# wjwei-handsome/wgatools

Measured on AMD Instinct MI355X. Metric: paf_cigar_ops_per_s (paf2maf+stat), higher is better.
Workload: dtype u8

## Files before the change

wgatools_amd/csrc/wga_intrin.h:

```cpp
#ifndef WGA_INTRIN_H
#define WGA_INTRIN_H

#ifdef WGA_EMU
#include "wga_intrin_emu.h"
#else

#define WGA_UNI32(x) ((u32)__builtin_amdgcn_readfirstlane((int)(x)))
#define WGA_UNI64(x)                                                               \
  (((u64)(u32)__builtin_amdgcn_readfirstlane((int)((u64)(x) >> 32)) << 32) |       \
   (u64)(u32)__builtin_amdgcn_readfirstlane((int)(u32)(u64)(x)))

#ifdef WGA_WAVE_ID_PLAIN
#define WGA_WAVE_ID(t) ((u32)(t) >> 6)
#else
#define WGA_WAVE_ID(t) ((u32)__builtin_amdgcn_readfirstlane((int)((u32)(t) >> 6)))
#endif

#define WGA_PIN(x) asm volatile("" : "+v"(x))
#define WGA_PIN4(a, b, c, d) asm volatile("" : "+v"(a), "+v"(b), "+v"(c), "+v"(d))
#define WGA_PIN7(a, b, c, d, e, f, g) asm volatile("" : "+v"(a), "+v"(b), "+v"(c), "+v"(d), "+v"(e), "+v"(f), "+v"(g))

__device__ __forceinline__ u32 wave_incl_scan_u32(u32 v) {
  v += (u32)__builtin_amdgcn_update_dpp(0, (int)v, 0x111, 0xF, 0xF, false);
  v += (u32)__builtin_amdgcn_update_dpp(0, (int)v, 0x112, 0xF, 0xF, false);
  v += (u32)__builtin_amdgcn_update_dpp(0, (int)v, 0x114, 0xF, 0xF, false);
  v += (u32)__builtin_amdgcn_update_dpp(0, (int)v, 0x118, 0xF, 0xF, false);
  v += (u32)__builtin_amdgcn_update_dpp(0, (int)v, 0x142, 0xA, 0xF, false);
  v += (u32)__builtin_amdgcn_update_dpp(0, (int)v, 0x143, 0xC, 0xF, false);
  return v;
}
__device__ __forceinline__ u32 wave_incl_scan_max_u32(u32 v) {
  u32 t;
  t = (u32)__builtin_amdgcn_update_dpp(0, (int)v, 0x111, 0xF, 0xF, false); v = v > t ? v : t;
  t = (u32)__builtin_amdgcn_update_dpp(0, (int)v, 0x112, 0xF, 0xF, false); v = v > t ? v : t;
  t = (u32)__builtin_amdgcn_update_dpp(0, (int)v, 0x114, 0xF, 0xF, false); v = v > t ? v : t;
  t = (u32)__builtin_amdgcn_update_dpp(0, (int)v, 0x118, 0xF, 0xF, false); v = v > t ? v : t;
  t = (u32)__builtin_amdgcn_update_dpp(0, (int)v, 0x142, 0xA, 0xF, false); v = v > t ? v : t;
  t = (u32)__builtin_amdgcn_update_dpp(0, (int)v, 0x143, 0xC, 0xF, false); v = v > t ? v : t;
  return v;
}
__device__ __forceinline__ u32 wave_shr1_u32(u32 v, u32 fill) {
  return (u32)__builtin_amdgcn_update_dpp((int)fill, (int)v, 0x138, 0xF, 0xF, false);
}
__device__ __forceinline__ u32 wave_last_u32(u32 incl) { return (u32)__builtin_amdgcn_readlane((int)incl, 63); }
template <u32 K>
__device__ __forceinline__ u64 lane_put_u64(u64 v, u64 uniform_val, u32 lane) {
  (void)lane;
  u32 lo = (u32)v, hi = (u32)(v >> 32);
  const u32 ulo = WGA_UNI32((u32)uniform_val), uhi = WGA_UNI32((u32)(uniform_val >> 32));
  asm("v_writelane_b32 %0, %1, %2" : "+v"(lo) : "s"(ulo), "n"(K));
  asm("v_writelane_b32 %0, %1, %2" : "+v"(hi) : "s"(uhi), "n"(K));
  return ((u64)hi << 32) | (u64)lo;
}

__device__ __forceinline__ u32 byte_perm(u32 hi, u32 lo, u32 sel) { return __builtin_amdgcn_perm(hi, lo, sel); }

#define WGA_BUF_OOB 0xFFFFFFFFu
typedef __amdgpu_buffer_rsrc_t BufRsrc;
typedef u32 u32x4_v __attribute__((vector_size(16)));
__device__ __forceinline__ BufRsrc buf_make(const void* base, u32 bytes) {
  const u64 b = (u64)base;
  const u32 lo = (u32)__builtin_amdgcn_readfirstlane((int)(u32)b);
  const u32 hi = (u32)__builtin_amdgcn_readfirstlane((int)(u32)(b >> 32));
  const u32 n = (u32)__builtin_amdgcn_readfirstlane((int)bytes);
  return __builtin_amdgcn_make_buffer_rsrc((void*)(((u64)hi << 32) | (u64)lo), (short)0, (int)n, 0x00020000);
}
__device__ __forceinline__ void buf_load16(const BufRsrc& r, u32 off, u32 v[4]) {
  const u32x4_v x = __builtin_amdgcn_raw_buffer_load_b128(r, (int)off, 0, 0);
  v[0] = x[0];
  v[1] = x[1];
  v[2] = x[2];
  v[3] = x[3];
}
#ifndef WGA_STORE_AUX
#define WGA_STORE_AUX 0
#endif
__device__ __forceinline__ void buf_store16(const BufRsrc& r, u32 off, const u32 v[4]) {
  const u32x4_v x = {v[0], v[1], v[2], v[3]};
  __builtin_amdgcn_raw_buffer_store_b128(x, r, (int)off, 0, WGA_STORE_AUX);
}
#ifndef WGA_STREAM_AUX
#define WGA_STREAM_AUX 2
#endif
__device__ __forceinline__ void buf_store16_stream(const BufRsrc& r, u32 off, const u32 v[4]) {
  const u32x4_v x = {v[0], v[1], v[2], v[3]};
  __builtin_amdgcn_raw_buffer_store_b128(x, r, (int)off, 0, WGA_STREAM_AUX);
}

__device__ __forceinline__ u64 wave_get_u64(u32 v, int k) {
  return (u64)(u32)__builtin_amdgcn_readlane((int)v, k) | ((u64)(u32)__builtin_amdgcn_readlane((int)v, k + 1) << 32);
}
__device__ __forceinline__ u32 wave_get_u32(u32 v, int k) { return (u32)__builtin_amdgcn_readlane((int)v, k); }
__device__ __forceinline__ u32 wave_get_u32_dyn(u32 v, u32 k) { return (u32)__builtin_amdgcn_readlane((int)v, (int)k); }
#define WGA_CLOCK() ((u64)__builtin_amdgcn_s_memtime())
#define WGA_SLEEP(n) __builtin_amdgcn_s_sleep(n)
#define WGA_WAVE_SYNC() __builtin_amdgcn_wave_barrier()

#ifndef WGA_MBCNT
#define WGA_MBCNT 1
#endif
__device__ __forceinline__ u32 lane_rank(u64 m, u32 lane) {
#if WGA_MBCNT
  (void)lane;
  return (u32)__builtin_amdgcn_mbcnt_hi((u32)(m >> 32), __builtin_amdgcn_mbcnt_lo((u32)m, 0u));
#else
  return (u32)__popcll(m & ((1ull << lane) - 1ull));
#endif
}

__device__ __forceinline__ u32x4_a16 ops_load16(const u32* p) {
#ifdef WGA_OPS_NT
  return __builtin_nontemporal_load((const u32x4_a16*)p);
#else
  return *(const u32x4_a16*)p;
#endif
}

__device__ __forceinline__ u32 bit_mask(u32 bits, u32 idx) { return (u32)__builtin_amdgcn_sbfe((int)bits, idx, 1u); }
__device__ __forceinline__ u32 bit_test(u32 bits, u32 idx) { return __builtin_amdgcn_ubfe(bits, idx, 1u); }

#define WGA_KARG_SPACE __attribute__((address_space(4)))
#define WGA_KARG_SEGMENT(T, a) ((T)__builtin_amdgcn_kernarg_segment_ptr())
#define WGA_KARG_FRESH(p) asm volatile("" : "+s"(p))

#ifndef WGA_W_STORE_AUX
#define WGA_W_STORE_AUX 2
#endif
__device__ __forceinline__ void buf_store16_w(const BufRsrc& r, u32 off, const u32 v[4]) {
  const u32x4_v x = {v[0], v[1], v[2], v[3]};
  __builtin_amdgcn_raw_buffer_store_b128(x, r, (int)off, 0, WGA_W_STORE_AUX);
}

__device__ __forceinline__ void lds_dma16(const void* gbase, u32 voff, void* lds_dst) {
  const u64 gb = WGA_UNI64((u64)gbase);
  const u32 ld = WGA_UNI32((u32)(u64)lds_dst);
  u32 keep;
  asm volatile("s_mov_b32 %0, m0\n\ts_mov_b32 m0, %3\n\ts_nop 0\n\tglobal_load_lds_dwordx4 %1, %2\n\ts_mov_b32 m0, %0"
               : "=&s"(keep)
               : "v"(voff), "s"(gb), "s"(ld)
               : "memory");
}
__device__ __forceinline__ void lds_dma16_after_reads(const void* gbase, u32 voff, void* lds_dst) {
  asm volatile("s_waitcnt lgkmcnt(0)" ::: "memory");
  lds_dma16(gbase, voff, lds_dst);
}
__device__ __forceinline__ void gstore16_nt(void* base, u32 voff, const u32 v[4]) {
  const u64 b = WGA_UNI64((u64)base);
  const u32x4_v x = {v[0], v[1], v[2], v[3]};
  asm volatile("global_store_dwordx4 %0, %1, %2 nt" ::"v"(voff), "v"(x), "s"(b) : "memory");
}
__device__ __forceinline__ void vm_wait(u32 k) {
  switch (k) {
    case 0: asm volatile("s_waitcnt vmcnt(0)" ::: "memory"); break;
    case 1: asm volatile("s_waitcnt vmcnt(1)" ::: "memory"); break;
    case 2: asm volatile("s_waitcnt vmcnt(2)" ::: "memory"); break;
    case 3: asm volatile("s_waitcnt vmcnt(3)" ::: "memory"); break;
    case 4: asm volatile("s_waitcnt vmcnt(4)" ::: "memory"); break;
    case 5: asm volatile("s_waitcnt vmcnt(5)" ::: "memory"); break;
    case 6: asm volatile("s_waitcnt vmcnt(6)" ::: "memory"); break;
    case 7: asm volatile("s_waitcnt vmcnt(7)" ::: "memory"); break;
    case 8: asm volatile("s_waitcnt vmcnt(8)" ::: "memory"); break;
    case 9: asm volatile("s_waitcnt vmcnt(9)" ::: "memory"); break;
    case 10: asm volatile("s_waitcnt vmcnt(10)" ::: "memory"); break;
    case 11: asm volatile("s_waitcnt vmcnt(11)" ::: "memory"); break;
    case 12: asm volatile("s_waitcnt vmcnt(12)" ::: "memory"); break;
    case 13: asm volatile("s_waitcnt vmcnt(13)" ::: "memory"); break;
    case 14: asm volatile("s_waitcnt vmcnt(14)" ::: "memory"); break;
    case 15: asm volatile("s_waitcnt vmcnt(15)" ::: "memory"); break;
    default: asm volatile("" ::: "memory"); break;
  }
}
__device__ __forceinline__ u32 bfi_b32(u32 mask, u32 a, u32 b) { return (a & mask) | (b & ~mask); }

#endif

struct wga_u64x2 {
  u64 x, y;
};
#if defined(__HIP_DEVICE_COMPILE__) && !defined(WGA_EMU)
#define WGA_RO_SPACE __attribute__((address_space(4)))
#define WGA_RO32(p) (*(const WGA_RO_SPACE u32*)(u64)(const u32*)(p))
#define WGA_RO64(p) (*(const WGA_RO_SPACE u64*)(u64)(const u64*)(p))
__device__ __forceinline__ wga_u64x2 wga_ro16(const u64* p) {
  typedef u64 u64x2_v __attribute__((vector_size(16)));
  const u64x2_v v = *(const WGA_RO_SPACE u64x2_v*)(u64)p;
  return {v[0], v[1]};
}
#define WGA_RO_HERE2(a, b) asm volatile("" ::"s"(a), "s"(b))
#define WGA_RO_HERE4(a, b, c, d) asm volatile("" ::"s"(a), "s"(b), "s"(c), "s"(d))
#else
#define WGA_RO32(p) (*(const u32*)(p))
#define WGA_RO64(p) (*(const u64*)(p))
__device__ __forceinline__ wga_u64x2 wga_ro16(const u64* p) { return {p[0], p[1]}; }
#define WGA_RO_HERE2(a, b) ((void)0)
#define WGA_RO_HERE4(a, b, c, d) ((void)0)
#endif

#endif
```

wgatools_amd/csrc/wga_kernels_k2s.h:

```cpp
#ifndef WGA_KERNELS_K2S_H
#define WGA_KERNELS_K2S_H

#include "wga_kernels.h"

#define WGA_S_FIFO 320u
#define WGA_S_MAX_JOB_TILES 32u
#define WGA_S_U 4u
#define WGA_S_WAVE_BYTES ((WGA_S_FIFO + 4u) * 8u + 1024u + 1024u + 256u + 272u + 16u)
#ifndef WGA_AUTO_LONG_VARIANT
#define WGA_AUTO_LONG_VARIANT 3
#endif

__global__ __launch_bounds__(256) void k_pseudo_rec_desc(u32 n, const wga_class_sums* sums, const u8* strand_neg, const u64* q_src_off,
                                                         const u64* q_src_len, const u64* skip, const u64* dst_off, const u64* op_off,
                                                         u64 q_fa_bytes, wga_rec_desc* out, u8* tile_flag) {
  const u32 r = blockIdx.x * 256u + threadIdx.x;
  if (r >= n) return;
  const wga_class_sums cs = sums[r];
  wga_rec_desc d;
  d.t_row_off = 0;
  d.q_row_off = dst_off[r] - skip[r];
  d.t_src_off = 0;
  d.t_src_len = skip[r];
  d.q_src_off = q_src_off ? q_src_off[r] : 0ull;
  d.q_src_len = q_src_len ? q_src_len[r] : 0ull;
  d.I_total = cs.i + cs.s;
  d.D_total = cs.d;
  d.L = cs.mx + cs.d;
  const bool clean = !q_src_len || d.q_src_len == cs.mx + cs.i + cs.s;
  const bool inside = !q_src_off || (d.q_src_off >= 32ull && d.q_src_off + d.q_src_len + 32ull <= q_fa_bytes);
  d.neg = (strand_neg[r] != 0 ? 1u : 0u) | (clean ? 0u : 8u);
  out[r] = d;
  if (clean && inside) return;
  const u64 a = op_off[r], b = op_off[r + 1];
  if (b <= a) return;
  for (u64 t = a / WGA_TILE; t <= (b - 1) / WGA_TILE; t++) tile_flag[t] = 1;
}

__device__ __forceinline__ u32 comp4s(u32 x, u32* bad) {
  const u32 sel = x & 0x07070707u;
  const u32 fold = byte_perm(0x474EFF54u, 0x43FF41FFu, sel);
  const u32 comp = byte_perm(0x434E0D41u, 0x47FF54FFu, sel);
  *bad = (x & 0xDFDFDFDFu) ^ fold;
  return comp | (x & 0x20202020u);
}

#define WGA_S_NOINLINE __forceinline__
__device__ WGA_S_NOINLINE void stream_store_bytes(u8* p, u32 o0, u32 o1, u32 o2, u32 o3, int lo, int hi) {
#pragma clang loop vectorize(disable) unroll(disable)
  for (int j = lo; j < hi; j++) {
    const u32 wj = j < 4 ? o0 : j < 8 ? o1 : j < 12 ? o2 : o3;
    p[j] = (u8)(wj >> (8 * (j & 3)));
  }
}
__device__ WGA_S_NOINLINE void stream_report_bad(u64* bad_base_pos, u32 b0, u32 b1, u32 b2, u32 b3, int lo, int hi, u32 Cl,
                                                 i64 Kseg, const u32* fifo, u32 k, u32 nf, u32 adj) {
#pragma clang loop vectorize(disable) unroll(disable)
  for (int j = lo; j < hi; j++) {
    const u32 bw = j < 4 ? b0 : j < 8 ? b1 : j < 12 ? b2 : b3;
    if (((bw >> (8 * (j & 3))) & 0xFFu) == 0u) continue;
    const u32 cj = Cl + (u32)j;
    u32 ad = adj;
    if (fifo) {
      u32 i = k - 1u;
      while (i + 1u < nf && (int)(fifo[2u * (i + 1u)] - cj) <= 0) i++;
      ad = fifo[2u * (i + 1u) + 1u];
    }
    atomicMin(bad_base_pos, (u64)((i64)(u64)(cj - ad) + Kseg));
  }
}

#define WGA_S_PSEUDO 2
#define WGA_S_SYMBOL 3
template <int MODE>
__device__ __forceinline__ u32 stream_glen(u32 c0, u32 c1) {
  return MODE == WGA_S_SYMBOL ? (c1 >> 1) - (c0 >> 1) : MODE == WGA_S_PSEUDO ? ((int)(c1 - c0) > 0 ? c1 - c0 : 0u) : c1 - c0;
}
__device__ __forceinline__ u32 stream_symbol(u32 cu) { return (cu & 1u) ? 0x2D2D2D2Du : 0x30303030u; }
template <int MODE>
__device__ __forceinline__ void stream_row(const ExpandArgs& a, u8* const lds, const u32 lane, const u64 job, const u64 t0,
                                           const u64 t1) {
  const u32 skipm = WGA_RO32(a.job_skip + job);
  u32* const s_fifo = (u32*)lds;
  u32x4_a16* const s_P = (u32x4_a16*)(s_fifo + 2u * (WGA_S_FIFO + 4u));
  u32* const s_q = (u32*)(s_P + 64);
  u32* const s_T = s_q + 256;
  u32x4_a16* const s_lm = (u32x4_a16*)(s_T + 64);
  u64* const s_k = (u64*)(s_lm + 17);
  if (lane < 17u) {
    u32x4_a16 m;
    for (int d = 0; d < 4; d++) m[d] = bytemask(0, (int)lane - 4 * d);
    s_lm[lane] = m;
  }
  constexpr bool QROW = MODE != 0;
  constexpr bool TCOORD = MODE >= WGA_S_PSEUDO;
  constexpr bool SYM = MODE == WGA_S_SYMBOL;
  constexpr u32 COL_MASK = TCOORD ? 0x585u : 0x787u;
  constexpr u32 GAP_MASK = MODE == 0 ? 0x202u : SYM ? 0x504u : 0x404u;
  constexpr u32 SKIP_MASK = MODE == WGA_S_PSEUDO ? 0x212u : 0u;
  const u8* const fa = QROW ? a.q_fa : a.t_fa;
  const u64 fa_bytes = QROW ? a.q_fa_bytes : a.t_fa_bytes;
  const u64 job_lo = t0 * WGA_TILE;
  const u32 q_end = WGA_UNI32((u32)((t1 * WGA_TILE < a.n_ops ? t1 * WGA_TILE : a.n_ops) - job_lo));
  const BufRsrc obuf = buf_make(a.ops + job_lo, (u32)(((a.n_ops - job_lo) < 0x3FFFFFFFull ? (a.n_ops - job_lo) : 0x3FFFFFFFull) * 4ull));

  u32 C_known = 0, cum_known = 0;
  u32 nf = 1;
  u32 e0 = 1;
  u32 pos = 0;
  u32 q = 0;
  u32 q_lo = 0, q_hi = 0;
  u32 rec = 0, re = 0;
  u8* dst_seg = nullptr;
  BufRsrc sbuf = buf_make(fa, 0u);
  u32 S32 = 0;
  bool rc = false;
  bool live = false;
  bool bnd = false;
  bool fin = false;
  u32 C_b = 0, cum_b = 0;
  u32 C_min = 0;
  u64 t = t0;
  u32 ow[4] = {0, 0, 0, 0}, xl0 = 0, xg0 = 0;
  u32 own[4] = {0, 0, 0, 0};

  auto fifo_dedupe = [&]() {
    WGA_WAVE_SYNC();
    u32 n_new = nf;
    if (lane == 0u) {
      u32 w = e0;
      for (u32 r = e0; r < nf; r++) {
        const u32 gs = s_fifo[2u * r], cu = s_fifo[2u * r + 1u];
        const bool dup = w > e0 && s_fifo[2u * (w - 1u)] == gs && (int)(cu - s_fifo[2u * (w - 1u) + 1u]) <= 0 &&
                         (int)(s_fifo[2u * (r + 1u) + 1u] - cu) <= 0;
        if (!dup) {
          s_fifo[2u * w] = gs;
          s_fifo[2u * w + 1u] = cu;
          w++;
        }
      }
      for (u32 k = 0; k < 3u; k++) {
        s_fifo[2u * (w + k)] = s_fifo[2u * (nf + k)];
        s_fifo[2u * (w + k) + 1u] = s_fifo[2u * (nf + k) + 1u];
      }
      n_new = w;
    }
    nf = wave_get_u32(n_new, 0);
    WGA_WAVE_SYNC();
  };

  for (;;) {
    {
      const u32 lim = bnd ? C_b : C_known;
      const bool all = bnd || fin;
      while ((int)(lim - pos) > 0) {
        if (TCOORD && (int)(C_min - pos) > 0) {
          const u32 to = (int)(lim - C_min) > 0 ? C_min : lim;
          u32 c;
          do {
            const u32 idx = e0 + lane < nf ? e0 + lane : nf;
            c = (u32)__popcll(__ballot(idx < nf && (int)(s_fifo[2u * idx] - to) < 0));
            e0 += c;
          } while (c == 64u);
          pos = to;
          continue;
        }
        u8* const A = dst_seg + pos;
        const u32 mis = (u32)(u64)A & 1023u;
        u8* const B = A - mis;
        const u32 room = WGA_S_U * 1024u - mis;
        if (!all && (lim - pos) < room) break;
        const u32 Cs = pos;
        u32 Ce = (lim - pos) < room ? lim : pos + room;
        const u32 Cl0 = Cs - mis;
        if (e0 + 255u < nf) {
          const u32 g255 = WGA_UNI32(s_fifo[2u * (e0 + 255u)]);
          if ((int)(g255 - Ce) < 0) Ce = Cl0 + ((g255 - Cl0) & ~15u);
          if (MODE == WGA_S_PSEUDO && (int)(Ce - Cs) < 16) {
            fifo_dedupe();
            continue;
          }
        }

        s_T[lane] = 0u;
        WGA_WAVE_SYNC();
        u32 nE = 0;
        {
          u32 base = e0, c;
          do {
            const u32 idx = base + lane < nf ? base + lane : nf;
            const u32 gsr = s_fifo[2u * idx] - Cl0;
            const bool in = gsr < Ce - Cl0;
            c = (u32)__popcll(__ballot(in));
            if (in) atomicAdd(&s_T[(gsr >> 4) & 63u], 1u << (8u * (gsr >> 10)));
            base += c;
            nE += c;
          } while (c == 64u);
        }
        WGA_WAVE_SYNC();
        const u32 tw = s_T[lane];
        WGA_WAVE_SYNC();
        const u32 tinc = wave_incl_scan_u32(tw);
        const u32 texc = tinc - tw;
        const u32 ttot = wave_last_u32(tinc);

        u32 kbase = e0;
        u32 qn = 0, rpk = 0, cls = 0;
        u32 adjv[WGA_S_U];
        const u32 wsp = Ce - Cs - 16u, asp = Ce - Cs + 15u;
        const bool any16 = (Ce - Cs) >= 16u;
        u32 qcum = 0;
#pragma unroll
        for (u32 u = 0; u < WGA_S_U; u++) {
          const u32 cnt = (tw >> (8u * u)) & 255u;
          const u32 k = kbase + ((texc >> (8u * u)) & 255u);
          kbase += (ttot >> (8u * u)) & 255u;
          const u32 Cl = Cl0 + 1024u * u + 16u * lane;
          const bool whole = any16 && (Cl - Cs) <= wsp, active = (Cl + 15u - Cs) < asp;
          const u32x4_a1 fe = *(const u32x4_a1*)(s_fifo + 2u * (k - 1u));
          const int rel0 = (int)(fe[0] + stream_glen<MODE>(fe[1], fe[3]) - Cl);
          const bool quiet = whole && cnt == 0u;
          const bool plain = quiet && rel0 <= 0;
          const bool dashes = quiet && rel0 >= 16;
          const bool flagged = active && !(plain || dashes);
          adjv[u] = fe[3];
          cls |= ((plain ? 1u : 0u) | (dashes ? 2u : 0u) | (flagged ? 4u : 0u) | (SYM ? (fe[1] & 1u) << 3 : 0u)) << (4u * u);
          const u64 m = __ballot(flagged);
          if (flagged) {
            const u32 r = qn + lane_rank(m, lane);
            s_q[r & 255u] = (k << 8) | (u << 6) | lane;
            rpk |= (r & 255u) << (8u * u);
          }
          qcum |= (qn > 255u ? 255u : qn) << (8u * u);
          qn += (u32)__popcll(m);
        }
        if (qn > 64u) {
          u32 keep = 1u;
#pragma unroll
          for (u32 u = 2; u <= WGA_S_U; u++) {
            const u32 upto = u == WGA_S_U ? qn : (qcum >> (8u * u)) & 255u;
            const bool sat = u < WGA_S_U && ((qcum >> (8u * u)) & 255u) == 255u;
            if (upto <= 64u && !sat) keep = u;
          }
          const u32 Cn = Cl0 + 1024u * keep;
          if ((int)(Cn - Ce) < 0) Ce = Cn;
          qn = keep == WGA_S_U ? qn : (qcum >> (8u * keep)) & 255u;
          nE = 0;
#pragma unroll
          for (u32 u = 0; u < WGA_S_U; u++)
            if (u < keep) nE += (ttot >> (8u * u)) & 255u;
        }
        const BufRsrc dbuf = buf_make(B, WGA_S_U * 1024u);

        WGA_WAVE_SYNC();
        if (lane < qn) {
          const u32 ent = s_q[lane];
          const u32 k = ent >> 8, Cl = Cl0 + 16u * (ent & 255u);
          int lo = (int)(Cs - Cl), hi = (int)(Ce - Cl);
          lo = lo < 0 ? 0 : (lo > 16 ? 16 : lo);
          hi = hi > 16 ? 16 : (hi < 0 ? 0 : hi);
          const u32x4_a1 ea = *(const u32x4_a1*)(s_fifo + 2u * (k - 1u));
          const u32x4_a1 eb = *(const u32x4_a1*)(s_fifo + 2u * (k + 1u));
          const u32 gs0 = ea[0], cu0 = ea[1], gs1 = ea[2], cu1 = ea[3], gs2 = eb[0], cu2 = eb[1];
          int a1 = (int)(gs0 + stream_glen<MODE>(cu0, cu1) - Cl);
          a1 = a1 < lo ? lo : (a1 > hi ? hi : a1);
          int b1 = (int)(gs1 - Cl);
          b1 = b1 < a1 ? a1 : (b1 > hi ? hi : b1);
          const u32 gl1 = stream_glen<MODE>(cu1, cu2);
          int e1 = gl1 >= 16u ? 16 : b1 + (int)gl1;
          e1 = e1 > hi ? hi : e1;
          bool more = (int)(gs2 - Cl) < hi;
          u32 W0[4], W1[4];
          if (!SYM) {
            buf_load16(sbuf, b1 > a1 ? (rc ? S32 - Cl + cu1 : S32 + Cl - cu1) : WGA_BUF_OOB, W0);
            buf_load16(sbuf, hi > e1 ? (rc ? S32 - Cl + cu2 : S32 + Cl - cu2) : WGA_BUF_OOB, W1);
          }
          const u32x4_a16 La = s_lm[a1], Lb = s_lm[b1], Le = s_lm[e1];
          u32 o[4], bad[4] = {0u, 0u, 0u, 0u};
#pragma unroll
          for (int d = 0; d < 4; d++) {
            if (SYM) {
              o[d] = bfi_b32(La[d], stream_symbol(cu0), bfi_b32(Le[d] & ~Lb[d], stream_symbol(cu1), 0x31313131u));
              continue;
            }
            u32 cp;
            if (rc)
              cp = comp4s(bfi_b32(Lb[d], bswap32(W0[3 - d]), bswap32(W1[3 - d])), &bad[d]);
            else
              cp = bfi_b32(Lb[d], W0[d], W1[d]);
            const u32 md = La[d] | (Le[d] & ~Lb[d]);
            o[d] = bfi_b32(md, 0x2D2D2D2Du, cp);
            bad[d] &= ~md;
          }
          u32 ie = k + 1u;
          while (more) {
            const u32 gsi = s_fifo[2u * ie], cui = s_fifo[2u * ie + 1u], gsn = s_fifo[2u * ie + 2u], cun = s_fifo[2u * ie + 3u];
            const int b = (int)(gsi - Cl);
            const u32 len = stream_glen<MODE>(cui, cun);
            const int e = len >= (u32)(hi - b) ? hi : b + (int)len;
            u32 W[4];
            if (SYM)
              W[0] = W[1] = W[2] = W[3] = 0x31313131u;
            else
              buf_load16(sbuf, rc ? S32 - Cl + cun : S32 + Cl - cun, W);
            const u32x4_a16 Mb = s_lm[b], Me = s_lm[e];
#pragma unroll
            for (int d = 0; d < 4; d++) {
              u32 x = W[d], bw = 0u;
              if (rc) x = comp4s(bswap32(W[3 - d]), &bw);
              if (SYM)
                o[d] = bfi_b32(Mb[d], o[d], bfi_b32(Me[d], stream_symbol(cui), x));
              else
                o[d] = bfi_b32(Mb[d], o[d], bfi_b32(Me[d], 0x2D2D2D2Du, x));
              bad[d] = (bad[d] & Mb[d]) | (bw & ~Me[d]);
            }
            ie++;
            more = (int)(gsn - Cl) < hi;
          }
          if (rc && (bad[0] | bad[1] | bad[2] | bad[3]) != 0u)
            stream_report_bad((u64*)&a.diag[rec].bad_base_pos, bad[0], bad[1], bad[2], bad[3], lo, hi, Cl, (i64)s_k[0], s_fifo, k, nf, 0u);
          const u32x4_a16 ov = {o[0], o[1], o[2], o[3]};
          s_P[lane] = ov;
        }
        WGA_WAVE_SYNC();

        u32 dat[WGA_S_U][4];
        const u32 wsp2 = Ce - Cs - 16u;
#pragma unroll
        for (u32 u = 0; u < WGA_S_U; u++) {
          const u32 Cl = Cl0 + 1024u * u + 16u * lane;
          const u32 c = (cls >> (4u * u)) & 15u;
          if (SYM) {
            dat[u][0] = dat[u][1] = dat[u][2] = dat[u][3] = (c & 2u) ? ((c & 8u) ? 0x2D2D2D2Du : 0x30303030u) : 0x31313131u;
            continue;
          }
          dat[u][0] = dat[u][1] = dat[u][2] = dat[u][3] = (c & 2u) ? 0x2D2D2D2Du : 0u;
          if ((c & 1u) && (int)(Cl - Ce) < 0) buf_load16(sbuf, rc ? S32 - Cl + adjv[u] : S32 + Cl - adjv[u], dat[u]);
        }
        if (rc) {
#pragma unroll
          for (u32 u = 0; u < WGA_S_U; u++) {
            u32 bad[4], x[4];
#pragma unroll
            for (int d = 0; d < 4; d++) x[d] = comp4s(bswap32(dat[u][3 - d]), &bad[d]);
#pragma unroll
            for (int d = 0; d < 4; d++) dat[u][d] = x[d];
            const u32 Cl = Cl0 + 1024u * u + 16u * lane;
            const bool pb = ((cls >> (4u * u)) & 1u) != 0u && (int)(Cl - Ce) < 0 && (bad[0] | bad[1] | bad[2] | bad[3]) != 0u;
            if (__ballot(pb)) {
              if (pb)
                stream_report_bad((u64*)&a.diag[rec].bad_base_pos, bad[0], bad[1], bad[2], bad[3], 0, 16, Cl, (i64)s_k[0], nullptr, 0u, 0u,
                                  adjv[u]);
            }
          }
        }
#pragma unroll
        for (u32 u = 0; u < WGA_S_U; u++) {
          const u32 Cl = Cl0 + 1024u * u + 16u * lane;
          const bool queued = ((cls >> (4u * u)) & 4u) != 0u && (int)(Cl - Ce) < 0;
          if (queued) {
            const u32x4_a16 pv = s_P[(rpk >> (8u * u)) & 255u];
            dat[u][0] = pv[0];
            dat[u][1] = pv[1];
            dat[u][2] = pv[2];
            dat[u][3] = pv[3];
          }
          const bool whole = (Ce - Cs) >= 16u && (Cl - Cs) <= wsp2;
          buf_store16_stream(dbuf, whole ? 1024u * u + 16u * lane : WGA_BUF_OOB, dat[u]);
          if (queued && !whole) {
            int lo = (int)(Cs - Cl), hi = (int)(Ce - Cl);
            lo = lo < 0 ? 0 : lo;
            hi = hi > 16 ? 16 : hi;
            stream_store_bytes(B + 1024u * u + lane * 16u, dat[u][0], dat[u][1], dat[u][2], dat[u][3], lo, hi);
          }
        }
        WGA_WAVE_SYNC();
        e0 += nE;
        pos = Ce;
      }
      fin = false;
    }

    if (bnd || !live) {
      const bool sw = bnd;
      u64 row_off, src_off, src_len, x_a, sb;
      bool neg;
      u32 C_a, cum_a;
      if (bnd) {
        const u64 bnd_op = job_lo + re;
        u64 ren, skip = 0;
        wga_u64x2 src;
        u32 negw;
        do {
          rec++;
          const wga_rec_desc* const rd = a.recs + rec;
          ren = WGA_RO64(a.op_off + rec + 1);
          row_off = WGA_RO64(QROW ? &rd->q_row_off : &rd->t_row_off);
          src = wga_ro16(QROW ? &rd->q_src_off : &rd->t_src_off);
          negw = WGA_RO32((const u32*)&rd->neg);
          if (TCOORD) skip = WGA_RO64(&rd->t_src_len);
          WGA_RO_HERE4(ren, row_off, src.x, src.y);
          WGA_RO_HERE2(negw, skip);
        } while (ren <= bnd_op);
        re = ren - job_lo > (u64)q_end ? q_end : (u32)(ren - job_lo);
        src_off = src.x;
        src_len = src.y;
        neg = (negw & 1u) != 0u;
        x_a = 0;
        sb = 0;
        C_a = C_b;
        cum_a = cum_b;
        if (TCOORD)
          C_min = C_a + (u32)(skip < 0x40000000ull ? skip : 0x40000000ull);
      } else {
        while (t < t1 && ((skipm >> (u32)(t - t0)) & 1u)) t++;
        if (t >= t1) break;
        const wga_tile_desc* const td = a.tdesc + t;
        const u64 tile_start = t * WGA_TILE;
        q = (u32)(tile_start - job_lo);
        WGA_WAVE_SYNC();
        C_known = cum_known = 0u;
        pos = 0u;
        nf = 1u;
        e0 = 1u;
        if (lane < 4u) {
          s_fifo[2u * lane] = 0u;
          s_fifo[2u * lane + 1u] = 0u;
        }
        rec = WGA_RO32(&td->rec);
        const u64 ren = WGA_RO64(&td->re), rs = WGA_RO64(&td->rs);
        const u64 d_mx = WGA_RO64(&td->b_mx), d_i = WGA_RO64(&td->b_i), d_d = WGA_RO64(&td->b_d);
        row_off = WGA_RO64(QROW ? &td->q_row_off : &td->t_row_off);
        src_off = WGA_RO64(QROW ? &td->q_src_off : &td->t_src_off);
        src_len = WGA_RO64(QROW ? &td->q_src_len : &td->t_src_len);
        neg = (WGA_RO32(&td->neg) & 1u) != 0u;
        const u64 skip = TCOORD ? WGA_RO64(&td->t_src_len) : 0ull;
        re = ren - job_lo > (u64)q_end ? q_end : (u32)(ren - job_lo);
        const bool cont = rs < tile_start;
        const u64 b_mx = cont ? d_mx : 0ull, b_i = cont ? d_i : 0ull, b_d = cont ? d_d : 0ull;
        x_a = TCOORD ? b_mx + b_d : b_mx + b_i + b_d;
        sb = QROW ? b_mx + b_i : b_mx + b_d;
        C_a = cum_a = 0u;
        if (TCOORD) {
          const u64 ahead = skip > x_a ? skip - x_a : 0ull;
          C_min = (u32)(ahead < 0x40000000ull ? ahead : 0x40000000ull);
        }
        buf_load16(obuf, q * 4u + lane * 16u, own);
        live = true;
      }
      dst_seg = (u8*)((u64)a.out + row_off + x_a - (u64)C_a);
      rc = QROW && !SYM && neg;
      const u32 adv = C_a - cum_a;
      u64 base;
      if (rc) {
        const u64 top = src_off + src_len;
        const u64 hiB = top > sb ? top - sb : 0ull;
        base = hiB > 0x60000000ull ? hiB - 0x60000000ull : 0ull;
        S32 = (u32)(top - base) - 16u - (u32)sb + adv;
      } else {
        const u64 loB = src_off + sb;
        base = loB > 64ull ? loB - 64ull : 0ull;
        S32 = (u32)(loB - base) - adv;
      }
      base = base > fa_bytes ? fa_bytes : base;
      {
        const u64 left = fa_bytes - base;
        sbuf = buf_make(fa + base, left > 0xFFFFFFF0ull ? 0xFFFFFFF0u : (u32)left);
      }
      if (lane == 0u) s_k[0] = (u64)((i64)sb - (i64)(u64)adv);
      WGA_WAVE_SYNC();
      bnd = false;
      if (sw && re < q_hi) {
        const u32 kb = re - q_lo, e = kb & 3u;
        u32 vl = xl0, vg = xg0;
#pragma unroll
        for (u32 i = 0; i < 3u; i++) {
          const bool valid = q_lo + 4u * lane + i < q_hi && i < e;
          const u32 len = valid ? ow[i] >> 4 : 0u, code = ow[i] & 15u;
          vl += len & bit_mask(COL_MASK, code);
          vg += (len & bit_mask(GAP_MASK, code)) - (len & bit_mask(SKIP_MASK, code));
        }
        C_b = wave_get_u32_dyn(vl, kb >> 2);
        cum_b = wave_get_u32_dyn(vg, kb >> 2);
        bnd = true;
      }
      continue;
    }

    if (q >= q_end) {
      if (pos != C_known) {
        fin = true;
        continue;
      }
      break;
    }
    if ((q & (WGA_TILE - 1u)) == 0u) {
      t = (job_lo + q) / WGA_TILE;
      if ((skipm >> (u32)(t - t0)) & 1u) {
        if (pos != C_known) {
          fin = true;
          continue;
        }
        live = false;
        t++;
        continue;
      }
    }
    if (e0 > 1u) {
      const u32 from = e0 - 1u, count = nf + 3u - from;
      for (u32 i0 = 0; i0 < count; i0 += 64u) {
        const u32 i = i0 + lane;
        u64 v = 0;
        if (i < count) v = *(const u64*)(s_fifo + 2u * (from + i));
        WGA_WAVE_SYNC();
        if (i < count) *(u64*)(s_fifo + 2u * i) = v;
        WGA_WAVE_SYNC();
      }
      nf -= from;
      e0 = 1u;
    }
    if (nf + 256u > WGA_S_FIFO) {
      fin = true;
      if (pos != C_known) continue;
      fin = false;
      if (MODE == WGA_S_PSEUDO) {
        fifo_dedupe();
        if (nf + 256u > WGA_S_FIFO) break;
      }
    }
    q_lo = q;
    q_hi = q + 256u < q_end ? q + 256u : q_end;
    q = q_hi;
    ow[0] = own[0], ow[1] = own[1], ow[2] = own[2], ow[3] = own[3];
    buf_load16(obuf, q_hi < q_end ? q_hi * 4u + lane * 16u : WGA_BUF_OOB, own);
    u32 l[4], g[4], sl = 0, sg = 0, sc = 0;
#pragma unroll
    for (int e = 0; e < 4; e++) {
      const bool valid = q_lo + 4u * lane + (u32)e < q_hi;
      const u32 len = valid ? ow[e] >> 4 : 0u, code = ow[e] & 15u;
      l[e] = len & bit_mask(COL_MASK, code);
      g[e] = (len & bit_mask(GAP_MASK, code)) - (len & bit_mask(SKIP_MASK, code));
      sl += l[e];
      sg += g[e];
      sc += g[e] != 0u ? 1u : 0u;
    }
    const u32 il = wave_incl_scan_u32(sl), ig = wave_incl_scan_u32(sg), ic = wave_incl_scan_u32(sc);
    xl0 = C_known + il - sl;
    xg0 = cum_known + ig - sg;
    {
      u32 xl = xl0, xg = xg0, xc = nf + ic - sc;
#pragma unroll
      for (int e = 0; e < 4; e++) {
        if (g[e] != 0u) {
          s_fifo[2u * xc] = xl;
          s_fifo[2u * xc + 1u] = SYM ? (xg << 1) | (bit_mask(0x404u, ow[e] & 15u) & 1u) : xg;
          xc++;
          xg += g[e];
        }
        xl += l[e];
      }
    }
    C_known += wave_last_u32(il);
    cum_known += wave_last_u32(ig);
    nf += wave_last_u32(ic);
    if (lane < 3u) {
      s_fifo[2u * (nf + lane)] = C_known;
      s_fifo[2u * (nf + lane) + 1u] = SYM ? cum_known << 1 : cum_known;
    }
    WGA_WAVE_SYNC();
    if (re < q_hi) {
      const u32 kb = re - q_lo, e = kb & 3u;
      u32 vl = xl0, vg = xg0;
#pragma unroll
      for (u32 i = 0; i < 3u; i++) {
        const bool valid = q_lo + 4u * lane + i < q_hi && i < e;
        const u32 len = valid ? ow[i] >> 4 : 0u, code = ow[i] & 15u;
        vl += len & bit_mask(COL_MASK, code);
        vg += (len & bit_mask(GAP_MASK, code)) - (len & bit_mask(SKIP_MASK, code));
      }
      C_b = wave_get_u32_dyn(vl, kb >> 2);
      cum_b = wave_get_u32_dyn(vg, kb >> 2);
      bnd = true;
    }
  }
}

__device__ __forceinline__ u64 xcd_job_of_block() {
  const u32 nb = gridDim.x, b = blockIdx.x, x = b & 7u, q = nb >> 3, r = nb & 7u;
  return (u64)(x * q + (x < r ? x : r) + (b >> 3));
}

__device__ __forceinline__ void expand_stream(const ExpandArgs& a) {
  __shared__ u32x4_a16 s_mem[2u * WGA_S_WAVE_BYTES / 16u];
  const u32 lane = threadIdx.x & 63u, wave = WGA_WAVE_ID(threadIdx.x);
  const u64 nt = (a.n_ops + WGA_TILE - 1) / WGA_TILE;
  const u64 job = xcd_job_of_block();
  const u64 t0 = job * a.job_tiles;
  if (t0 >= nt) return;
  const u64 t1 = t0 + a.job_tiles < nt ? t0 + a.job_tiles : nt;
  u8* const lds = (u8*)s_mem + wave * WGA_S_WAVE_BYTES;
  if (wave == 0u)
    stream_row<0>(a, lds, lane, job, t0, t1);
  else
    stream_row<1>(a, lds, lane, job, t0, t1);
}
template <int MODE>
__device__ __forceinline__ void pseudo_stream(const ExpandArgs& a) {
  __shared__ u32x4_a16 s_mem[2u * WGA_S_WAVE_BYTES / 16u];
  const u32 lane = threadIdx.x & 63u, wave = WGA_WAVE_ID(threadIdx.x);
  const u64 nt = (a.n_ops + WGA_TILE - 1) / WGA_TILE;
  const u64 job = 2u * xcd_job_of_block() + wave;
  const u64 t0 = job * a.job_tiles;
  if (t0 >= nt) return;
  const u64 t1 = t0 + a.job_tiles < nt ? t0 + a.job_tiles : nt;
  stream_row<MODE>(a, (u8*)s_mem + wave * WGA_S_WAVE_BYTES, lane, job, t0, t1);
}
#ifndef WGA_S_WAVES_PER_SIMD
#define WGA_S_WAVES_PER_SIMD 5
#endif
__global__ __launch_bounds__(128, WGA_S_WAVES_PER_SIMD) void k_paf2maf_expand_s(ExpandArgs a) { expand_stream(a); }
__global__ __launch_bounds__(128, WGA_S_WAVES_PER_SIMD) void k_pafpseudo_stream(ExpandArgs a) { pseudo_stream<WGA_S_PSEUDO>(a); }
#ifndef WGA_S_SYM_WAVES
#define WGA_S_SYM_WAVES 5
#endif
__global__ __launch_bounds__(128, WGA_S_SYM_WAVES) void k_pafpseudo_stream_sym(ExpandArgs a) { pseudo_stream<WGA_S_SYMBOL>(a); }

#endif
```

Baseline: 86.38 billion.

## Park next op block in LDS and batch sequence loads ahead of cut processing

The next 256-op CIGAR block is no longer held in registers across iterations. It is fetched inside the emit step and parked in a double-buffered LDS slot, so the load overlaps the emit work and register pressure drops. Source-sequence loads for the per-tile data and the cut windows are issued together before the cut-handling code, with a partial vmcnt wait, so more memory requests are in flight at once. The emit loop becomes a do-while around a step_due predicate, and the boundary recompute reuses the already-decoded lengths. This adds LDS use per wave, extra waits and more complex control flow.

```diff
diff --git a/wgatools_amd/csrc/wga_intrin.h b/wgatools_amd/csrc/wga_intrin.h
--- a/wgatools_amd/csrc/wga_intrin.h
+++ b/wgatools_amd/csrc/wga_intrin.h
@@ -188,12 +188,21 @@
 }
 #define WGA_RO_HERE2(a, b) asm volatile("" ::"s"(a), "s"(b))
 #define WGA_RO_HERE4(a, b, c, d) asm volatile("" ::"s"(a), "s"(b), "s"(c), "s"(d))
+#define WGA_VM_LANDED() __builtin_amdgcn_s_waitcnt(0x0F70)
+#define WGA_VM_LEFT6() __builtin_amdgcn_s_waitcnt(0x0F76)
 #else
 #define WGA_RO32(p) (*(const u32*)(p))
 #define WGA_RO64(p) (*(const u64*)(p))
 __device__ __forceinline__ wga_u64x2 wga_ro16(const u64* p) { return {p[0], p[1]}; }
 #define WGA_RO_HERE2(a, b) ((void)0)
 #define WGA_RO_HERE4(a, b, c, d) ((void)0)
-#endif
-
-#endif
+#define WGA_VM_LANDED() ((void)0)
+#define WGA_VM_LEFT6() ((void)0)
+#endif
+#if defined(__HIP_DEVICE_COMPILE__) && !defined(WGA_EMU)
+#define WGA_GLOBAL_STORE_U8(p, v) (*(__attribute__((address_space(1))) u8*)(p) = (v))
+#else
+#define WGA_GLOBAL_STORE_U8(p, v) (*(u8*)(p) = (v))
+#endif
+
+#endif
diff --git a/wgatools_amd/csrc/wga_kernels_k2s.h b/wgatools_amd/csrc/wga_kernels_k2s.h
--- a/wgatools_amd/csrc/wga_kernels_k2s.h
+++ b/wgatools_amd/csrc/wga_kernels_k2s.h
@@ -6,7 +6,7 @@
 #define WGA_S_FIFO 320u
 #define WGA_S_MAX_JOB_TILES 32u
 #define WGA_S_U 4u
-#define WGA_S_WAVE_BYTES ((WGA_S_FIFO + 4u) * 8u + 1024u + 1024u + 256u + 272u + 16u)
+#define WGA_S_WAVE_BYTES ((WGA_S_FIFO + 4u) * 8u + 1024u + 1024u + 256u + 272u + 16u + 2u * 1024u)
 #ifndef WGA_AUTO_LONG_VARIANT
 #define WGA_AUTO_LONG_VARIANT 3
 #endif
@@ -50,7 +50,7 @@
 #pragma clang loop vectorize(disable) unroll(disable)
   for (int j = lo; j < hi; j++) {
     const u32 wj = j < 4 ? o0 : j < 8 ? o1 : j < 12 ? o2 : o3;
-    p[j] = (u8)(wj >> (8 * (j & 3)));
+    WGA_GLOBAL_STORE_U8(p + j, (u8)(wj >> (8 * (j & 3))));
   }
 }
 __device__ WGA_S_NOINLINE void stream_report_bad(u64* bad_base_pos, u32 b0, u32 b1, u32 b2, u32 b3, int lo, int hi, u32 Cl,
@@ -87,6 +87,7 @@
   u32* const s_T = s_q + 256;
   u32x4_a16* const s_lm = (u32x4_a16*)(s_T + 64);
   u64* const s_k = (u64*)(s_lm + 17);
+  u32x4_a16* const s_ow = (u32x4_a16*)(s_k + 2);
   if (lane < 17u) {
     u32x4_a16 m;
     for (int d = 0; d < 4; d++) m[d] = bytemask(0, (int)lane - 4 * d);
@@ -121,8 +122,9 @@
   u32 C_b = 0, cum_b = 0;
   u32 C_min = 0;
   u64 t = t0;
-  u32 ow[4] = {0, 0, 0, 0}, xl0 = 0, xg0 = 0;
-  u32 own[4] = {0, 0, 0, 0};
+  u32 xl0 = 0, xg0 = 0;
+  u32 par = 0;
+  bool parked = true;
 
   auto fifo_dedupe = [&]() {
     WGA_WAVE_SYNC();
@@ -153,7 +155,12 @@
     {
       const u32 lim = bnd ? C_b : C_known;
       const bool all = bnd || fin;
-      while ((int)(lim - pos) > 0) {
+      auto step_due = [&]() -> bool {
+        if ((int)(lim - pos) <= 0) return false;
+        if (TCOORD && (int)(C_min - pos) > 0) return true;
+        return all || (lim - pos) >= WGA_S_U * 1024u - ((u32)(u64)(dst_seg + pos) & 1023u);
+      };
+      if (step_due()) do {
         if (TCOORD && (int)(C_min - pos) > 0) {
           const u32 to = (int)(lim - C_min) > 0 ? C_min : lim;
           u32 c;
@@ -169,7 +176,6 @@
         const u32 mis = (u32)(u64)A & 1023u;
         u8* const B = A - mis;
         const u32 room = WGA_S_U * 1024u - mis;
-        if (!all && (lim - pos) < room) break;
         const u32 Cs = pos;
         u32 Ce = (lim - pos) < room ? lim : pos + room;
         const u32 Cl0 = Cs - mis;
@@ -181,6 +187,10 @@
             continue;
           }
         }
+
+        const bool fetch = !parked;
+        u32 own[4];
+        buf_load16(obuf, fetch && q < q_end ? q * 4u + lane * 16u : WGA_BUF_OOB, own);
 
         s_T[lane] = 0u;
         WGA_WAVE_SYNC();
@@ -253,7 +263,11 @@
         const BufRsrc dbuf = buf_make(B, WGA_S_U * 1024u);
 
         WGA_WAVE_SYNC();
-        if (lane < qn) {
+        const bool mq = lane < qn;
+        u32 cuts = 0;
+        u32 W0[4], W1[4];
+        u32 off0 = WGA_BUF_OOB, off1 = WGA_BUF_OOB;
+        if (mq) {
           const u32 ent = s_q[lane];
           const u32 k = ent >> 8, Cl = Cl0 + 16u * (ent & 255u);
           int lo = (int)(Cs - Cl), hi = (int)(Ce - Cl);
@@ -269,12 +283,39 @@
           const u32 gl1 = stream_glen<MODE>(cu1, cu2);
           int e1 = gl1 >= 16u ? 16 : b1 + (int)gl1;
           e1 = e1 > hi ? hi : e1;
-          bool more = (int)(gs2 - Cl) < hi;
-          u32 W0[4], W1[4];
-          if (!SYM) {
-            buf_load16(sbuf, b1 > a1 ? (rc ? S32 - Cl + cu1 : S32 + Cl - cu1) : WGA_BUF_OOB, W0);
-            buf_load16(sbuf, hi > e1 ? (rc ? S32 - Cl + cu2 : S32 + Cl - cu2) : WGA_BUF_OOB, W1);
-          }
+          if (b1 > a1) off0 = rc ? S32 - Cl + cu1 : S32 + Cl - cu1;
+          if (hi > e1) off1 = rc ? S32 - Cl + cu2 : S32 + Cl - cu2;
+          cuts = (u32)a1 | ((u32)b1 << 8) | ((u32)e1 << 16) | ((int)(gs2 - Cl) < hi ? 1u << 24 : 0u);
+        }
+        if (!SYM) {
+          buf_load16(sbuf, off0, W0);
+          buf_load16(sbuf, off1, W1);
+        }
+        u32 dat[WGA_S_U][4];
+        const u32 wsp2 = Ce - Cs - 16u;
+        if (!SYM) {
+#pragma unroll
+          for (u32 u = 0; u < WGA_S_U; u++) {
+            const u32 Cl = Cl0 + 1024u * u + 16u * lane;
+            const bool pl = ((cls >> (4u * u)) & 1u) != 0u && (int)(Cl - Ce) < 0;
+            buf_load16(sbuf, pl ? (rc ? S32 - Cl + adjv[u] : S32 + Cl - adjv[u]) : WGA_BUF_OOB, dat[u]);
+          }
+        }
+        if (!SYM) WGA_VM_LEFT6();
+        if (!SYM && fetch) {
+          const u32x4_a16 nx = {own[0], own[1], own[2], own[3]};
+          s_ow[64u * (par ^ 1u) + lane] = nx;
+          parked = true;
+        }
+        if (mq) {
+          const u32 ent = s_q[lane];
+          const u32 k = ent >> 8, Cl = Cl0 + 16u * (ent & 255u);
+          int lo = (int)(Cs - Cl), hi = (int)(Ce - Cl);
+          lo = lo < 0 ? 0 : (lo > 16 ? 16 : lo);
+          hi = hi > 16 ? 16 : (hi < 0 ? 0 : hi);
+          const u32 cu0 = s_fifo[2u * (k - 1u) + 1u], cu1 = s_fifo[2u * k + 1u];
+          const int a1 = (int)(cuts & 255u), b1 = (int)((cuts >> 8) & 255u), e1 = (int)((cuts >> 16) & 255u);
+          bool more = (cuts >> 24) != 0u;
           const u32x4_a16 La = s_lm[a1], Lb = s_lm[b1], Le = s_lm[e1];
           u32 o[4], bad[4] = {0u, 0u, 0u, 0u};
 #pragma unroll
@@ -324,18 +365,16 @@
         }
         WGA_WAVE_SYNC();
 
-        u32 dat[WGA_S_U][4];
-        const u32 wsp2 = Ce - Cs - 16u;
 #pragma unroll
         for (u32 u = 0; u < WGA_S_U; u++) {
-          const u32 Cl = Cl0 + 1024u * u + 16u * lane;
           const u32 c = (cls >> (4u * u)) & 15u;
           if (SYM) {
             dat[u][0] = dat[u][1] = dat[u][2] = dat[u][3] = (c & 2u) ? ((c & 8u) ? 0x2D2D2D2Du : 0x30303030u) : 0x31313131u;
             continue;
           }
-          dat[u][0] = dat[u][1] = dat[u][2] = dat[u][3] = (c & 2u) ? 0x2D2D2D2Du : 0u;
-          if ((c & 1u) && (int)(Cl - Ce) < 0) buf_load16(sbuf, rc ? S32 - Cl + adjv[u] : S32 + Cl - adjv[u], dat[u]);
+          const u32 dash = (c & 2u) ? 0x2D2D2D2Du : 0u;
+#pragma unroll
+          for (int d = 0; d < 4; d++) dat[u][d] |= dash;
         }
         if (rc) {
 #pragma unroll
@@ -353,6 +392,11 @@
                                   adjv[u]);
             }
           }
+        }
+        if (SYM && fetch) {
+          const u32x4_a16 nx = {own[0], own[1], own[2], own[3]};
+          s_ow[64u * (par ^ 1u) + lane] = nx;
+          parked = true;
         }
 #pragma unroll
         for (u32 u = 0; u < WGA_S_U; u++) {
@@ -377,6 +421,14 @@
         WGA_WAVE_SYNC();
         e0 += nE;
         pos = Ce;
+      } while (step_due());
+      if (!parked) {
+        u32 own[4];
+        buf_load16(obuf, q < q_end ? q * 4u + lane * 16u : WGA_BUF_OOB, own);
+        WGA_VM_LANDED();
+        const u32x4_a16 nx = {own[0], own[1], own[2], own[3]};
+        s_ow[64u * (par ^ 1u) + lane] = nx;
+        parked = true;
       }
       fin = false;
     }
@@ -445,7 +497,7 @@
           const u64 ahead = skip > x_a ? skip - x_a : 0ull;
           C_min = (u32)(ahead < 0x40000000ull ? ahead : 0x40000000ull);
         }
-        buf_load16(obuf, q * 4u + lane * 16u, own);
+        parked = false;
         live = true;
       }
       dst_seg = (u8*)((u64)a.out + row_off + x_a - (u64)C_a);
@@ -473,6 +525,7 @@
       if (sw && re < q_hi) {
         const u32 kb = re - q_lo, e = kb & 3u;
         u32 vl = xl0, vg = xg0;
+        const u32x4_a16 ow = s_ow[64u * par + lane];
 #pragma unroll
         for (u32 i = 0; i < 3u; i++) {
           const bool valid = q_lo + 4u * lane + i < q_hi && i < e;
@@ -531,8 +584,9 @@
     q_lo = q;
     q_hi = q + 256u < q_end ? q + 256u : q_end;
     q = q_hi;
-    ow[0] = own[0], ow[1] = own[1], ow[2] = own[2], ow[3] = own[3];
-    buf_load16(obuf, q_hi < q_end ? q_hi * 4u + lane * 16u : WGA_BUF_OOB, own);
+    par ^= 1u;
+    parked = false;
+    const u32x4_a16 ow = s_ow[64u * par + lane];
     u32 l[4], g[4], sl = 0, sg = 0, sc = 0;
 #pragma unroll
     for (int e = 0; e < 4; e++) {
@@ -573,10 +627,8 @@
       u32 vl = xl0, vg = xg0;
 #pragma unroll
       for (u32 i = 0; i < 3u; i++) {
-        const bool valid = q_lo + 4u * lane + i < q_hi && i < e;
-        const u32 len = valid ? ow[i] >> 4 : 0u, code = ow[i] & 15u;
-        vl += len & bit_mask(COL_MASK, code);
-        vg += (len & bit_mask(GAP_MASK, code)) - (len & bit_mask(SKIP_MASK, code));
+        vl += i < e ? l[i] : 0u;
+        vg += i < e ? g[i] : 0u;
       }
       C_b = wave_get_u32_dyn(vl, kb >> 2);
       cum_b = wave_get_u32_dyn(vg, kb >> 2);
```

Measured after the change: 88.73 billion (median of 6 runs). 1.03x the previous value.
